# robjermy/CMVS-PMVS

Hardware: AMD Instinct MI355X
Metric: refined patches/sec + NCC evals/sec, 50-view 4K synthetic, 1/2/4/8 GPU (higher is better)
Workload: dtype f32 (f64 optimizer)

## Files before the change

cmvs-pmvs_amd/csrc/bobyqa_dev.h:

```cpp
#pragma once

#if defined(__HIPCC__)
#define BQ_HD __host__ __device__ inline __attribute__((always_inline))
#else
#define BQ_HD inline
#endif
#if defined(__HIP_DEVICE_COMPILE__) && defined(BQ_PRIVATE)
#define BQ_AS __attribute__((address_space(5)))
#elif defined(__HIP_DEVICE_COMPILE__)
#define BQ_AS __attribute__((address_space(3)))
#else
#define BQ_AS
#endif
#if defined(__HIPCC__) && !defined(BQ_INLINE)
#define BQ_NI __host__ __device__ inline __attribute__((noinline))
#else
#define BQ_NI BQ_HD
#endif

#include <math.h>

#if defined(BQ_NO_RESTRICT)
#define BQ_RS
#else
// ... 37 lines not shown
BQ_HD double bq_min(double a, double b) { return (a <= b) ? a : b; }
BQ_HD double bq_max(double a, double b) { return (a >= b) ? a : b; }
template <int N>
BQ_HD double bq_get(const double (&a)[N], int i) {
  double r = a[0];
#pragma unroll
  for (int k = 1; k < N; ++k) r = (i == k) ? a[k] : r;
  return r;
}
template <int N>
BQ_HD void bq_set(double (&a)[N], int i, double v) {
#pragma unroll
  for (int k = 0; k < N; ++k) a[k] = (i == k) ? v : a[k];
}

struct BqState {
  double x_[BQN], xl_[BQN], xu_[BQN], s[BQN];
  double rhobeg, rhoend;
  int maxeval, nevals;
  double xbase_[BQN], xpt_[BQNPT][BQN], fval_[BQNPT], xopt_[BQN], gopt_[BQN], hq_[BQNH], pq_[BQNPT],
      bmat_[BQNDIM][BQN], zmat_[BQNPT][BQNPTM], sl_[BQN], su_[BQN], xnew_[BQN], xalt_[BQN], d_[BQN],
      vlag_[BQNDIM], w_[BQNDIM + BQNPT];
  double gnew_[BQN];
  double ptsaux_[2][BQN], ptsid_[BQNPT];
  double f, fbeg, fsave, xoptsq, rho, delta, diffa, diffb, diffc, dnorm, distsq, dsq, crvmin,
      adelt, alpha, cauchy, beta, denom, fopt, vquad, diff, ratio, stepa, stepb;
  int nf, kopt, kbase, nresc, ntrits, itest, nfsav, knew;
  int nfm, nfx, kpt, rs_ip, rs_iq;
  double rs_xp, rs_xq, rs_vq, rs_fbase;
  int rc;
  int resume;
  double xeval[BQN];
  double xout[BQN];
  double minf;
};

#define BQ_A1(name) BQ_AS double* const name = (st).name##_ - 1
#define BQ_A2(name, C) BQ_AS double(*const name)[C] = (BQ_AS double(*)[C])(&(st).name##_[0][0] - (C) - 1)
#define BQ_ALIASES(st)                                                                                         \
  BQ_A1(x); BQ_A1(xl); BQ_A1(xu); BQ_A1(xbase); BQ_A1(fval); BQ_A1(xopt); BQ_A1(gopt); BQ_A1(hq); BQ_A1(pq); \
  BQ_A1(sl); BQ_A1(su); BQ_A1(xnew); BQ_A1(xalt); BQ_A1(d); BQ_A1(vlag); BQ_A1(w); BQ_A1(gnew); BQ_A1(ptsid); \
  BQ_A2(xpt, BQN); BQ_A2(bmat, BQN); BQ_A2(zmat, BQNPTM); BQ_A2(ptsaux, BQN)

BQ_NI void bq_trsbox(const BQ_AS double (*BQ_RST xpt)[BQN], const BQ_AS double* BQ_RST xopt_m, const BQ_AS double* BQ_RST gopt,
                     const BQ_AS double* BQ_RST hq_m, const BQ_AS double* BQ_RST pq_m, const BQ_AS double* BQ_RST sl_m,
                     const BQ_AS double* BQ_RST su_m, double delta, BQ_AS double* BQ_RST xnew, BQ_AS double* BQ_RST d_m,
                     BQ_AS double* BQ_RST gnew_m, BQ_AS double* BQ_RST dsq_out, BQ_AS double* BQ_RST crvmin_out) {
  const double half = 0.5, one = 1.0, onemin = -1.0, zero = 0.0;
#if !defined(BQ_TRSBOX_LDS)
  double xopt[BQN + 1], hq[BQNH + 1], pq[BQNPT + 1], sl[BQN + 1], su[BQN + 1], d[BQN + 1], gnew[BQN + 1];
  for (int k = 1; k <= BQNPT; ++k) pq[k] = pq_m[k];
  for (int i = 1; i <= BQNH; ++i) hq[i] = hq_m[i];
  for (int i = 1; i <= BQN; ++i) {
    xopt[i] = xopt_m[i];
    sl[i] = sl_m[i];
    su[i] = su_m[i];
  }
// ... 550 lines not shown

BQ_HD double bq_default_step(double x, double lb, double ub) {
  double step = HUGE_VAL;
  if (!isinf(ub) && !isinf(lb) && (ub - lb) * 0.25 < step && ub > lb) step = (ub - lb) * 0.25;
  if (!isinf(ub) && ub - x < step && ub > x) step = (ub - x) * 0.75;
  if (!isinf(lb) && x - lb < step && x > lb) step = (x - lb) * 0.75;
  if (isinf(step)) {
    if (!isinf(ub) && fabs(ub - x) < fabs(step)) step = (ub - x) * 1.1;
    if (!isinf(lb) && fabs(x - lb) < fabs(step)) step = (x - lb) * 1.1;
  }
  if (isinf(step) || step == 0.0 || fabs(step) < 2.2250738585072014e-308) step = x;
  if (isinf(step) || step == 0.0) step = 1;
  return step;
}

BQ_HD int bq_begin(BQ_AS BqState& st, const double* x0, const double* lb, const double* ub,
                   double xtol_rel, int maxeval) {
  BQ_ALIASES(st);
  double dxs[BQN];
  for (int i = 0; i < BQN; ++i) dxs[i] = bq_default_step(x0[i], lb[i], ub[i]);
  for (int i = 0; i < BQN; ++i) st.s[i] = 1.0;
  {
    int i = 1;
    for (; i < BQN && dxs[i] == dxs[i - 1]; ++i) {
    }
    if (i < BQN)
      for (i = 1; i < BQN; ++i) st.s[i] = dxs[i] / dxs[0];
  }
  for (int i = 0; i < BQN; ++i) {
    x[i + 1] = x0[i] / st.s[i];
    xl[i + 1] = lb[i] / st.s[i];
    xu[i + 1] = ub[i] / st.s[i];
  }
  st.rhobeg = fabs(dxs[0] / st.s[0]);
  st.rhoend = xtol_rel * st.rhobeg;
  st.maxeval = maxeval;
  st.nevals = 0;
  st.rc = BQR_SUCCESS;
  st.resume = 0;
  st.minf = 0;
  for (int j = 1; j <= BQN; ++j) {
    const double temp = xu[j] - xl[j];
    if (temp < st.rhobeg + st.rhobeg) {
      st.rc = BQR_INVALID_ARGS;
      for (int i = 0; i < BQN; ++i) st.xout[i] = x0[i];
      st.resume = -1;
      return BQR_INVALID_ARGS;
    }
    sl[j] = xl[j] - x[j];
    su[j] = xu[j] - x[j];
    if (sl[j] >= -st.rhobeg) {
      if (sl[j] >= 0.0) {
        x[j] = xl[j];
        sl[j] = 0.0;
        su[j] = temp;
      } else {
        x[j] = xl[j] + st.rhobeg;
        sl[j] = -st.rhobeg;
        su[j] = bq_max(xu[j] - x[j], st.rhobeg);
      }
    } else if (su[j] <= st.rhobeg) {
      if (su[j] <= 0.0) {
        x[j] = xu[j];
        sl[j] = -temp;
        su[j] = 0.0;
      } else {
        x[j] = xu[j] - st.rhobeg;
        sl[j] = bq_min(xl[j] - x[j], -st.rhobeg);
        su[j] = st.rhobeg;
      }
    }
  }
  return 0;
}

#define BQ_CALFUN(P, LABEL_ID)                                             \
  do {                                                                     \
    for (int i_ = 0; i_ < BQN; ++i_) st.xeval[i_] = (P)[i_ + 1] * st.s[i_]; \
    st.nevals++;                                                           \
    st.resume = LABEL_ID;                                                  \
    return BQ_NEED_F;                                                      \
  } while (0)

BQ_NI int bq_step_impl(BQ_AS BqState& st, double fin);
BQ_HD int bq_step(BQ_AS BqState& st, double fin) {
  BQ_PT(t_all);
  const int r = bq_step_impl(st, fin);
  BQ_PA(3, t_all);
  return r;
}
BQ_NI int bq_step_impl(BQ_AS BqState& st, double fin) {
  BQ_ALIASES(st);
  const double half = 0.5, one = 1.0, ten = 10.0, tenth = 0.1, two = 2.0, zero = 0.0;
  double temp, sum, suma, sumb, bsum, dx, delsq, scaden, biglsq, hdiag, den, errbig, frhosq,
      bdtol, bdtest, curv, fracsq, sumpq, sumz, sumw, densav, pqold, gqsq, gisq, dist;
  int ih, ksav;
  switch (st.resume) {
    case 0: goto PSTART;
    case 1: goto PRESUME;
    case 2: goto L360R;
    case 3: goto R260R;
    default: return BQ_DONE;
  }
PSTART: {
    for (int j = 1; j <= BQN; ++j) {
      xbase[j] = x[j];
      for (int k = 1; k <= BQNPT; ++k) xpt[k][j] = zero;
      for (int i = 1; i <= BQNDIM; ++i) bmat[i][j] = zero;
    }
    for (int i = 1; i <= BQNH; ++i) hq[i] = zero;
    for (int k = 1; k <= BQNPT; ++k) {
      pq[k] = zero;
      for (int j = 1; j <= BQNPTM; ++j) zmat[k][j] = zero;
    }
    st.nf = 0;
    st.kopt = 1;
  PLOOP:
    st.nfm = st.nf;
    st.nfx = st.nf - BQN;
    ++st.nf;
    if (st.nfm <= 2 * BQN) {
      if (st.nfm >= 1 && st.nfm <= BQN) {
        st.stepa = st.rhobeg;
        if (su[st.nfm] == zero) st.stepa = -st.stepa;
        xpt[st.nf][st.nfm] = st.stepa;
      } else if (st.nfm > BQN) {
        st.stepa = xpt[st.nf - BQN][st.nfx];
        st.stepb = -st.rhobeg;
        if (sl[st.nfx] == zero) st.stepb = bq_min(two * st.rhobeg, su[st.nfx]);
        if (su[st.nfx] == zero) st.stepb = bq_max(-two * st.rhobeg, sl[st.nfx]);
        xpt[st.nf][st.nfx] = st.stepb;
      }
    }
    for (int j = 1; j <= BQN; ++j) {
      x[j] = bq_min(bq_max(xl[j], xbase[j] + xpt[st.nf][j]), xu[j]);
      if (xpt[st.nf][j] == sl[j]) x[j] = xl[j];
      if (xpt[st.nf][j] == su[j]) x[j] = xu[j];
    }
    BQ_CALFUN(x, 1);
  }
PRESUME: {
    const double rhosq = st.rhobeg * st.rhobeg;
    const int nf = st.nf, nfm = st.nfm, nfx = st.nfx;
    st.f = fin;
    fval[nf] = st.f;
    if (nf == 1) {
      st.fbeg = st.f;
      st.kopt = 1;
    } else if (st.f < fval[st.kopt]) {
      st.kopt = nf;
    }
    if (nf <= 2 * BQN + 1) {
      if (nf >= 2 && nf <= BQN + 1) {
        gopt[nfm] = (st.f - st.fbeg) / st.stepa;
        if (BQNPT < nf + BQN) {
          bmat[1][nfm] = -one / st.stepa;
          bmat[nf][nfm] = one / st.stepa;
          bmat[BQNPT + nfm][nfm] = -half * rhosq;
        }
      } else if (nf >= BQN + 2) {
        ih = nfx * (nfx + 1) / 2;
        temp = (st.f - st.fbeg) / st.stepb;
        st.diff = st.stepb - st.stepa;
        hq[ih] = two * (temp - gopt[nfx]) / st.diff;
        gopt[nfx] = (gopt[nfx] * st.stepb - temp * st.stepa) / st.diff;
        if (st.stepa * st.stepb < zero) {
          if (st.f < fval[nf - BQN]) {
            fval[nf] = fval[nf - BQN];
            fval[nf - BQN] = st.f;
            if (st.kopt == nf) st.kopt = nf - BQN;
            xpt[nf - BQN][nfx] = st.stepb;
            xpt[nf][nfx] = st.stepa;
          }
        }
        bmat[1][nfx] = -(st.stepa + st.stepb) / (st.stepa * st.stepb);
        bmat[nf][nfx] = -half / xpt[nf - BQN][nfx];
        bmat[nf - BQN][nfx] = -bmat[1][nfx] - bmat[nf][nfx];
        zmat[1][nfx] = sqrt(two) / (st.stepa * st.stepb);
        zmat[nf][nfx] = sqrt(half) / rhosq;
        zmat[nf - BQN][nfx] = -zmat[1][nfx] - zmat[nf][nfx];
      }
    }
    if (st.maxeval > 0 && st.nevals >= st.maxeval) {
      st.rc = BQR_MAXEVAL;
    } else if (st.nf < BQNPT) {
      goto PLOOP;
    }
  }
  st.xoptsq = zero;
  for (int i = 1; i <= BQN; ++i) {
    xopt[i] = xpt[st.kopt][i];
    st.xoptsq += xopt[i] * xopt[i];
  }
  st.fsave = fval[1];
  if (st.rc != BQR_SUCCESS) goto L720;
  st.kbase = 1;
  st.rho = st.rhobeg;
  st.delta = st.rho;
  st.nresc = st.nf;
  st.ntrits = 0;
  st.diffa = zero;
  st.diffb = zero;
  st.diffc = zero;
  st.ratio = zero;
  st.itest = 0;
  st.nfsav = st.nf;
  st.knew = 0;
L20:
  if (st.kopt != st.kbase) {
    ih = 0;
    for (int j = 1; j <= BQN; ++j) {
      for (int i = 1; i <= j; ++i) {
// ... 139 lines not shown
    for (int j = 1; j <= BQN; ++j) {
      xbase[j] += xopt[j];
      sl[j] -= xopt[j];
      su[j] -= xopt[j];
      xopt[j] = zero;
      ptsaux[1][j] = bq_min(st.delta, su[j]);
      ptsaux[2][j] = bq_max(-st.delta, sl[j]);
      if (ptsaux[1][j] + ptsaux[2][j] < zero) {
        temp = ptsaux[1][j];
        ptsaux[1][j] = ptsaux[2][j];
        ptsaux[2][j] = temp;
      }
      if (fabs(ptsaux[2][j]) < half * fabs(ptsaux[1][j])) ptsaux[2][j] = half * ptsaux[1][j];
      for (int i = 1; i <= BQNDIM; ++i) bmat[i][j] = zero;
    }
    st.rs_fbase = fval[st.kopt];
    ptsid[1] = sfrac;
    for (int j = 1; j <= BQN; ++j) {
      const int jp = j + 1, jpn = jp + BQN;
      ptsid[jp] = (double)j + sfrac;
      if (jpn <= BQNPT) {
        ptsid[jpn] = (double)j / (double)BQNP + sfrac;
        temp = one / (ptsaux[1][j] - ptsaux[2][j]);
        bmat[jp][j] = -temp + one / ptsaux[1][j];
        bmat[jpn][j] = temp + one / ptsaux[2][j];
        bmat[1][j] = -bmat[jp][j] - bmat[jpn][j];
        zmat[1][j] = sqrt(2.) / fabs(ptsaux[1][j] * ptsaux[2][j]);
        zmat[jp][j] = zmat[1][j] * ptsaux[2][j] * temp;
        zmat[jpn][j] = -zmat[1][j] * ptsaux[1][j] * temp;
      } else {
        bmat[1][j] = -one / ptsaux[1][j];
// ... 91 lines not shown
        den = bet2 * hdiag + vlag[k] * vlag[k];
        if (den > den2) {
          kold = k;
          den2 = den;
        }
      }
      vlmxsq = bq_max(vlmxsq, vlag[k] * vlag[k]);
    }
    if (den2 <= vlmxsq * .01) {
      w[BQNDIM + kn] = -w[BQNDIM + kn] - winc;
      goto R120;
    }
    goto R80;
  }
R260:
  st.kpt = 1;
R260LOOP:
  if (st.kpt > BQNPT) goto R350;
  if (ptsid[st.kpt] == zero) {
    ++st.kpt;
    goto R260LOOP;
  }
  if (st.maxeval > 0 && st.nevals >= st.maxeval) {
    st.nf = -1;
    goto R350;
  }
  {
    const int kpt = st.kpt;
    ih = 0;
    for (int j = 1; j <= BQN; ++j) {
      w[j] = xpt[kpt][j];
      xpt[kpt][j] = zero;
      temp = pq[kpt] * w[j];
      for (int i = 1; i <= j; ++i) {
        ++ih;
        hq[ih] += temp * w[i];
      }
    }
    pq[kpt] = zero;
    st.rs_ip = (int)ptsid[kpt];
    st.rs_iq = (int)((double)BQNP * ptsid[kpt] - (double)(st.rs_ip * BQNP));
    const int ip = st.rs_ip, iq = st.rs_iq;
    int ihp = 0, ihq;
    if (ip > 0) {
      st.rs_xp = ptsaux[1][ip];
      xpt[kpt][ip] = st.rs_xp;
    }
    if (iq > 0) {
      st.rs_xq = ptsaux[1][iq];
      if (ip == 0) st.rs_xq = ptsaux[2][iq];
      xpt[kpt][iq] = st.rs_xq;
    }
    st.rs_vq = st.rs_fbase;
    if (ip > 0) {
      ihp = (ip + ip * ip) / 2;
      st.rs_vq += st.rs_xp * (gopt[ip] + half * st.rs_xp * hq[ihp]);
    }
    if (iq > 0) {
      ihq = (iq + iq * iq) / 2;
      st.rs_vq += st.rs_xq * (gopt[iq] + half * st.rs_xq * hq[ihq]);
      if (ip > 0) {
        const int iw = (ihp > ihq ? ihp : ihq) - (ip > iq ? ip - iq : iq - ip);
        st.rs_vq += st.rs_xp * st.rs_xq * hq[iw];
      }
    }
    for (int k = 1; k <= BQNPT; ++k) {
      temp = zero;
      if (ip > 0) temp += st.rs_xp * xpt[k][ip];
      if (iq > 0) temp += st.rs_xq * xpt[k][iq];
      st.rs_vq += half * pq[k] * temp * temp;
    }
    for (int i = 1; i <= BQN; ++i) {
      w[i] = bq_min(bq_max(xl[i], xbase[i] + xpt[kpt][i]), xu[i]);
      if (xpt[kpt][i] == sl[i]) w[i] = xl[i];
      if (xpt[kpt][i] == su[i]) w[i] = xu[i];
    }
    ++st.nf;
    BQ_CALFUN(w, 3);
  }
R260R: {
    const int kpt = st.kpt, ip0 = st.rs_ip, iq0 = st.rs_iq;
    (void)ip0; (void)iq0;
    st.f = fin;
    fval[kpt] = st.f;
    if (st.f < fval[st.kopt]) st.kopt = kpt;
    st.diff = st.f - st.rs_vq;
    for (int i = 1; i <= BQN; ++i) gopt[i] += st.diff * bmat[kpt][i];
    for (int k = 1; k <= BQNPT; ++k) {
      sum = zero;
      for (int j = 1; j <= BQNPTM; ++j) sum += zmat[k][j] * zmat[kpt][j];
      temp = st.diff * sum;
      if (ptsid[k] == zero) {
        pq[k] += temp;
      } else {
        const int ip = (int)ptsid[k];
        const int iq = (int)((double)BQNP * ptsid[k] - (double)(ip * BQNP));
        const int ihq = (iq * iq + iq) / 2;
        if (ip == 0) {
          hq[ihq] += temp * (ptsaux[2][iq] * ptsaux[2][iq]);
        } else {
          const int ihp = (ip * ip + ip) / 2;
          hq[ihp] += temp * (ptsaux[1][ip] * ptsaux[1][ip]);
          if (iq > 0) {
            hq[ihq] += temp * (ptsaux[1][iq] * ptsaux[1][iq]);
            const int iw = (ihp > ihq ? ihp : ihq) - (iq > ip ? iq - ip : ip - iq);
            hq[iw] += temp * ptsaux[1][ip] * ptsaux[1][iq];
          }
        }
      }
    }
    ptsid[kpt] = zero;
    ++st.kpt;
    goto R260LOOP;
  }
R350:
  st.xoptsq = zero;
  if (st.kopt != st.kbase) {
    for (int i = 1; i <= BQN; ++i) {
      xopt[i] = xpt[st.kopt][i];
      st.xoptsq += xopt[i] * xopt[i];
    }
  }
  if (st.nf < 0) {
    st.nf = st.maxeval;
    st.rc = BQR_MAXEVAL;
    goto L720;
  }
// ... 99 lines not shown
    if (xnew[i] == sl[i]) x[i] = xl[i];
    if (xnew[i] == su[i]) x[i] = xu[i];
  }
  if (st.maxeval > 0 && st.nevals >= st.maxeval) {
    st.rc = BQR_MAXEVAL;
    goto L720;
  }
  ++st.nf;
  BQ_CALFUN(x, 2);
L360R:
  st.f = fin;
  if (st.ntrits == -1) {
    st.fsave = st.f;
    st.rc = BQR_XTOL;
    if (st.fsave < fval[st.kopt]) {
      st.minf = st.f;
      for (int i = 0; i < BQN; ++i) st.xout[i] = x[i + 1] * st.s[i];
      st.resume = -1;
      return BQ_DONE;
    }
    goto L720;
  }
  st.fopt = fval[st.kopt];
  st.vquad = zero;
  ih = 0;
  for (int j = 1; j <= BQN; ++j) {
    st.vquad += d[j] * gopt[j];
    for (int i = 1; i <= j; ++i) {
      ++ih;
      temp = d[i] * d[j];
      if (i == j) temp = half * temp;
      st.vquad += hq[ih] * temp;
// ... 195 lines not shown
    st.ntrits = 0;
    st.nfsav = st.nf;
    goto L60;
  }
  if (st.ntrits == -1) goto L360;
  st.rc = BQR_XTOL;
L720:
  if (fval[st.kopt] <= st.fsave) {
    for (int i = 1; i <= BQN; ++i) {
      x[i] = bq_min(bq_max(xl[i], xbase[i] + xopt[i]), xu[i]);
      if (xopt[i] == sl[i]) x[i] = xl[i];
      if (xopt[i] == su[i]) x[i] = xu[i];
    }
    st.f = fval[st.kopt];
  }
  st.minf = st.f;
  for (int i = 0; i < BQN; ++i) st.xout[i] = x[i + 1] * st.s[i];
  st.resume = -1;
  return BQ_DONE;
}

#undef BQ_CALFUN

}
```

cmvs-pmvs_amd/csrc/pmvs_api.cpp:

```cpp
#include <hip/hip_runtime.h>

#include <algorithm>
#include <climits>
#include <cmath>
#include <cstdarg>
#include <cstdio>
#include <cstdlib>
#include <cstring>
#include <chrono>
#include <condition_variable>
#include <mutex>
#include <string>
#include <vector>

#include "../../include/pmvs_amd.h"
#include "pmvs_features.h"
#include "pmvs_fmt.h"
#include "pmvs_launch.h"

using namespace pmvsdev;

namespace {

thread_local std::string g_err = "";
// ... 125 lines not shown
  DScene ds{};
  int maxLevel = 0;
  std::vector<DView> hviews;
  DevBuf<DView> views;
  DevBuf<uint32_t> pyr;
  DevBuf<uint8_t> masks, edges;
  DevBuf<int> vis_off, vis, bindexes;
  DevBuf<float> scratch;
  DevBuf<DevStats> stats;
  DevBuf<RefineJob> jobs;
  FilterBuffers fbuf;
  ExpandBuffers xbuf;
  DevBuf<pmvs_patch> fpatches;
  DevBuf<int> fkeep;
  DevBuf<unsigned long long> digest;
  int grid = 0, refine_grid = 0, tslots = 226014;
  int tslots_small = 300000, small_n = 7000;
  int refine_cfg(int n) const { return n < small_n ? tslots_small : tslots; }
  int shard_rank = 0, shard_world = 1;
  pmvs_allgather_fn shard_fn = nullptr;
  void* shard_ctx = nullptr;
  pmvs_rccl* shard_rccl = nullptr;
  int cl_rank = 0, cl_world = 1;
  pmvs_allgather_fn cl_fn = nullptr;
  void* cl_ctx = nullptr;
  pmvs_rccl* cl_rccl = nullptr;
  DevBuf<unsigned char> cl_shared;
  DevBuf<int> cl_ids, cl_id2idx;
  int cl_maxid = -1;
  ClusterBuffers cbuf;
  RefineHost rhost;
// ... 1631 lines not shown
```

cmvs-pmvs_amd/csrc/pmvs_kernels.hip:

```cpp
#include <hip/hip_runtime.h>

#include <algorithm>
#include <cmath>
#include <condition_variable>
#include <functional>
#include <mutex>
#include <thread>
#include <unistd.h>
#include <vector>

#include "bobyqa_dev.h"
#include "pmvs_device.h"
#include "pmvs_refine.h"

namespace pmvsdev {

#ifndef REFINE_TSLOTS
#define REFINE_TSLOTS 48
#endif

typedef uint16_t img_t;

template <int WS>
struct WaveLds {
// ... 1664 lines not shown
    if ((e = launch_refine_lane(tslots, s, d_jobs, n, d_st, stream)) != hipSuccess) return e;
    if (refine_tail_on()) hipLaunchKernelGGL(refine_tail_kernel, dim3(1), dim3(64), 0, stream, d_st, 1);
    (void)hipEventRecord(ev[2], stream);
    hipLaunchKernelGGL((post_kernel<WS>), dim3(g), dim3(64), 0, stream, s, d_jobs, d_out, n, d_st);
    (void)hipEventRecord(ev[3], stream);
    return hipGetLastError();
  }
  if (tslots >= 200000 && tslots < 300000 && WS > 7) tslots = 1206;
  if (tslots / 100 < s.tau) {
    tslots = 2408;
    refine_grid = refine_grid / 2 > 0 ? refine_grid / 2 : 1;
  }
  const int nc = tslots % 100;
  const int rg = refine_grid < (n + nc - 1) / nc ? refine_grid : (n + nc - 1) / nc;
  if (tslots >= 200000) {
    if ((e = launch_refine_split(tslots, s, d_jobs, n, d_st, stream)) != hipSuccess) return e;
    if (refine_tail_on()) hipLaunchKernelGGL(refine_tail_kernel, dim3(1), dim3(64), 0, stream, d_st, 0);
    (void)hipEventRecord(ev[2], stream);
    hipLaunchKernelGGL((post_kernel<WS>), dim3(g), dim3(64), 0, stream, s, d_jobs, d_out, n, d_st);
    (void)hipEventRecord(ev[3], stream);
    dump_jobs(d_jobs, n, stream);
    return hipGetLastError();
  }
  if (tslots >= 100000) {
    const int ncw = (tslots / 1000) % 100, wgpc = tslots % 10;
    int dev = 0, cus = 0;
    if ((e = hipGetDevice(&dev)) != hipSuccess ||
        (e = hipDeviceGetAttribute(&cus, hipDeviceAttributeMultiprocessorCount, dev)) != hipSuccess)
      return e;
    cus = cus > 0 ? cus : 1;
    const int wgrid = cus * wgpc < n ? cus * wgpc : n;
// ... 408 lines not shown
```

cmvs-pmvs_amd/csrc/pmvs_launch.h:

```cpp
#pragma once
#include <hip/hip_runtime.h>
#include "pmvs_device.h"
#include "pmvs_devbuf.h"
#include <functional>
#include <memory>
#include <utility>
#include <vector>

namespace pmvsdev {

inline hipError_t memset_big(void* p, int value, size_t bytes, hipStream_t st) {
  constexpr size_t kPiece = size_t(1) << 30;
  char* c = static_cast<char*>(p);
  for (size_t off = 0; off < bytes; off += kPiece) {
    const hipError_t e = hipMemsetAsync(c + off, value, bytes - off < kPiece ? bytes - off : kPiece, st);
    if (e != hipSuccess) return e;
  }
  return hipSuccess;
}
bool refine_config_supported(int tslots);
struct RefineHost {
  float4* d_enc = nullptr;
  double2* d_ang = nullptr;
  float4* h_enc = nullptr;
  double2* h_ang = nullptr;
  size_t cap = 0;
  bool prof = false;
  hipEvent_t ev_pre = nullptr;
  double trip_ms = 0.0;
  long long trips = 0;
  hipError_t ensure(size_t n);
  void release();
  ~RefineHost() { release(); }
};
int prepost_waves();
hipError_t launch_refine(const DScene& s, const pmvs_candidate* d_in, RefineJob* d_jobs, pmvs_refined* d_out, int n,
                         DevStats* d_st, int grid, int refine_grid, int tslots, hipStream_t stream, hipEvent_t* ev,
                         RefineHost& rh);
bool refine_split_supported(int config);
hipError_t launch_refine_split(int config, const DScene& s, RefineJob* d_jobs, int n, DevStats* d_st, hipStream_t stream);
bool refine_lane_supported(int config);
hipError_t launch_refine_lane(int config, const DScene& s, RefineJob* d_jobs, int n, DevStats* d_st, hipStream_t stream);
hipError_t launch_incc_eval(const DScene& s, const pmvs_eval_query* d_q, int n, double* d_out, DevStats* d_st,
                            hipStream_t stream);
hipError_t launch_grab_tex(const DScene& s, const pmvs_tex_query* d_q, int n, float* d_out, int* d_valid,
                           hipStream_t stream);
hipError_t launch_build_level(const uint8_t* d_src, int Wp, int Hp, uint8_t* d_dst, int W, int H, hipStream_t stream);
hipError_t launch_pack_rgba(const uint8_t* d_rgb, uint32_t* d_out, long long npix, hipStream_t stream);
hipError_t launch_unpack_rgba(const uint32_t* d_in, uint8_t* d_rgb, long long npix, hipStream_t stream);
hipError_t launch_math_selftest(int op, const double* d_in, double* d_out, int n, hipStream_t stream);
hipError_t launch_bobyqa_selftest(int mode, int kind, const double* d_x0, int n, int maxeval, double* d_out,
                                  hipStream_t stream);
hipError_t launch_model_digest(const void* recs, int n, int record_bytes, unsigned long long* d_out, hipStream_t stream);
hipError_t launch_patch_colors(const DScene& s, int n, const float* coords, const int* off, const int* images, int* out,
                               hipStream_t stream);
// ... 216 lines not shown
```

cmvs-pmvs_amd/csrc/pmvs_refine_split.hip:

```cpp
#include <hip/hip_runtime.h>

#include "bobyqa_dev.h"
#include "pmvs_device.h"
#include "pmvs_launch.h"
#include "pmvs_refine.h"

namespace pmvsdev {

#if defined(BQ_PROFILE)
#define SP_NOW() __builtin_amdgcn_s_memtime()
#define SP_MARK(slot)                                      \
  do {                                                     \
    const unsigned long long _t = __builtin_amdgcn_s_memtime(); \
    prof[slot] += _t - tprev;                              \
    tprev = _t;                                            \
  } while (0)
#else
#define SP_NOW() 0ull
#define SP_MARK(slot) \
  do {                \
  } while (0)
#endif

#ifndef SPLIT_WPE
#define SPLIT_WPE 2
#endif
#ifndef SPLIT_THREADS_
#define SPLIT_THREADS_ 512
#endif
constexpr int SPLIT_THREADS = SPLIT_THREADS_;
constexpr int SPLIT_TS = 64;

template <int WS, int G, int CG>
struct RefSplitLds {
  static constexpr int NCH = G * CG;
  static constexpr int SLOTS = CG * PMVS_MAX_TAU;
  BqState bq[NCH];
  float geo[NCH][16];
  double fv[NCH];
  int cand[NCH];
  unsigned short views[NCH][PMVS_MAX_TAU];
  unsigned char need[NCH], size[NCH];
  unsigned char sreq[G][SLOTS], sidx[G][SLOTS];
  short choff[G][CG + 1];
  int nchunk[G];
  int avail[G], done[G];
  int live;
  int ejvalid[8][SPLIT_TS];
  float ejres[8][SPLIT_TS];
};

#define SPLIT_AS __attribute__((address_space(3)))
// ... 186 lines not shown
    C.fv[cc] = request_value(s, V, t, C.size[cc], need, jobs[C.cand[cc]], tex_valid);
  }
  SP_MARK(6);
  __builtin_amdgcn_fence(__ATOMIC_RELEASE, "workgroup");
  if (lane == 0) __hip_atomic_fetch_add(&C.done[g], 1, __ATOMIC_RELEASE, __HIP_MEMORY_SCOPE_WORKGROUP);
  return tex_valid;
}
template <int WS, int G, int CG, int LP>
__device__ __noinline__ unsigned long long split_chunk(const DScene& s, SPLIT_AS RefSplitLds<WS, G, CG>& C,
                                                       RefineJob* __restrict__ jobs, int g, int k, unsigned long long* prof) {
  return split_chunk_body<WS, G, CG, LP>(s, C, jobs, g, k, prof);
}

template <int WS, int G, int CG, int LP>
__device__ __noinline__ void split_optimizer(const DScene& s, SPLIT_AS RefSplitLds<WS, G, CG>& C, RefineJob* __restrict__ jobs,
                                             int n, int nc_active, DevStats* st) {
  constexpr int TS = WAVE / LP;
  const int wave = threadIdx.x >> 6, lane = threadIdx.x & (WAVE - 1);
  const int g = wave;
  const bool owner = lane < CG && lane < nc_active;
  const int c = g * CG + (lane < CG ? lane : 0);
  BQ_AS BqState& bq = *(BQ_AS BqState*)&C.bq[c];
  RefineSetup R;
  int cand = -1, need = 0, evals = 0, size = 0, nimg = 0, rc = 0;
  bool exhausted = !owner;
  double fv = 0.0;
  float fcoord[4], fnormal[4];
  unsigned long long nevals = 0, rounds = 0, tex_valid = 0, grabs = 0, chunks = 0;
  const double lb[3] = {-HUGE_VAL, -23.99999, -23.99999};
  const double ub[3] = {HUGE_VAL, 23.99999, 23.99999};
  unsigned long long prof[8] = {0, 0, 0, 0, 0, 0, 0, 0};
  unsigned long long tprev = SP_NOW();
  for (;;) {
    while (cand < 0 && !exhausted) {
      const unsigned long long q = atomicAdd(&st->queue2, 1ull);
      if (q >= (unsigned long long)n) {
        exhausted = true;
// ... 1 lines not shown
        break;
      }
      const RefineJob& J = jobs[q];
      if (J.status != PMVS_ACCEPTED) continue;
      cand = (int)q;
      for (int i = 0; i < 4; ++i) { R.center[i] = J.center[i]; R.ray[i] = J.ray[i]; }
      R.dscale = J.dscale;
      R.ascale = s.ascale;
      R.ref = J.images[0];
      nimg = J.nimg;
      size = imin(s.tau, nimg);
      for (int i = 0; i < size; ++i) C.views[c][i] = (unsigned short)J.images[i];
      C.cand[c] = cand;
      evals = 0;
      const double x0[3] = {J.x0[0], J.x0[1], J.x0[2]};
      bq_begin(bq, x0, lb, ub, 1.e-7, 1000);
      fv = 0.0;
      need = 0;
    }
    SP_MARK(0);
    if (cand >= 0 && need == 0) {
      const int r = (bq.resume < 0) ? BQ_DONE : bq_step(bq, fv);
      if (r == BQ_NEED_F) {
        need = 1;
        const double xe[3] = {bq.xeval[0], bq.xeval[1], bq.xeval[2]};
        decode(s, R, xe, fcoord, fnormal);
      } else {
        rc = bq.rc;
        const bool success = (rc == BQR_SUCCESS || rc == 2 || rc == 3 || rc == BQR_XTOL);
        RefineJob& J = jobs[cand];
        J.refine_code = rc;
        J.evals = evals;
        if (success) {
          const double xo[3] = {bq.xout[0], bq.xout[1], bq.xout[2]};
          decode(s, R, xo, fcoord, fnormal);
          if (nimg < 2) {
            J.ncc = (float)(1.0 - (double)unrobustincc(2.0f));
            for (int i = 0; i < 4; ++i) { J.rcoord[i] = fcoord[i]; J.rnormal[i] = fnormal[i]; }
            cand = -1;
          } else {
            need = 2;
          }
        } else {
          cand = -1;
        }
      }
    }
    SP_MARK(1);
    const bool req = (cand >= 0 && need != 0);
// ... 129 lines not shown
  }
  SP_MARK(7);
  for (int d = 32; d >= 1; d >>= 1) tex_valid += __shfl_xor(tex_valid, d);
  if (lane == 0) {
#if defined(BQ_PROFILE)
    for (int i = 4; i < 8; ++i) atomicAdd(&st->prof[i], prof[i]);
#endif
    atomicAdd(&st->tex_valid, tex_valid);
    atomicAdd(&st->tex_grabs, grabs);
    atomicAdd(&st->chunks, chunks);
  }
}

template <int WS, int G, int CG, int LP>
__global__ __launch_bounds__(SPLIT_THREADS) __attribute__((amdgpu_waves_per_eu(SPLIT_WPE))) void refine_split_kernel(
    DScene s, RefineJob* __restrict__ jobs, int n, int nc_active, DevStats* st) {
  using L = RefSplitLds<WS, G, CG>;
  static_assert(G >= 1 && G <= SPLIT_THREADS / WAVE && CG <= WAVE && CG <= 255, "roles");
  static_assert(sizeof(L) <= 160 * 1024, "LDS");
  __shared__ L C;
  const int tid = threadIdx.x, wave = tid >> 6;
  if (tid < G) {
    C.avail[tid] = 0;
    C.done[tid] = 0;
    C.nchunk[tid] = 0;
  }
  if (tid == 0) {
    C.live = G;
    atomicMax(&st->t_first_inv, ~__builtin_amdgcn_s_memrealtime());
  }
  __syncthreads();
  if (wave < G)
    split_optimizer<WS, G, CG, LP>(s, *(SPLIT_AS RefSplitLds<WS, G, CG>*)&C, jobs, n, nc_active, st);
  else
    split_evaluator<WS, G, CG, LP>(s, *(SPLIT_AS RefSplitLds<WS, G, CG>*)&C, jobs, st);
}


#if SPLIT_THREADS_ == 512
#define PMVS_SPLIT_CONFIGS(X) X(0, 2, 32) X(0, 4, 16) X(2, 4, 16) X(2, 5, 16) X(2, 6, 12) X(2, 6, 14) X(2, 7, 12) \
  X(2, 8, 10) X(3, 6, 14) X(4, 5, 16) X(4, 6, 14) X(4, 7, 12) X(4, 8, 10) X(8, 8, 10)
#else
#define PMVS_SPLIT_CONFIGS(X) X(2, 4, 20) X(4, 4, 20) X(8, 4, 20) X(2, 2, 40) X(4, 3, 24)
#endif
bool refine_split_supported(int config) {
#define PMVS_SPLIT_CASE(LPc, Gc, CGc) case 200000 + LPc * 10000 + Gc * 1000 + CGc:
  switch (config) {
    PMVS_SPLIT_CONFIGS(PMVS_SPLIT_CASE)
    return true;
    default: return false;
  }
#undef PMVS_SPLIT_CASE
}

template <int WS>
static hipError_t launch_split_ws(int config, const DScene& s, RefineJob* d_jobs, int n, DevStats* d_st, hipStream_t stream) {
  const int gw = (config / 1000) % 10, cg = config % 1000;
  int dev = 0, cus = 0;
  hipError_t e;
  if ((e = hipGetDevice(&dev)) != hipSuccess ||
      (e = hipDeviceGetAttribute(&cus, hipDeviceAttributeMultiprocessorCount, dev)) != hipSuccess)
    return e;
  cus = cus > 0 ? cus : 1;
  const int sgrid = cus < (n + gw - 1) / gw ? cus : (n + gw - 1) / gw;
  const int per = (n + sgrid * gw - 1) / (sgrid * gw);
  const int nca = per < cg ? per : cg;
#define PMVS_SPLIT_LAUNCH(LPc, Gc, CGc)                                                                                   \
  case 200000 + LPc * 10000 + Gc * 1000 + CGc:                                                                             \
    hipLaunchKernelGGL((refine_split_kernel<WS, Gc, CGc, (LPc > 0 ? LPc : 1)>), dim3(sgrid), dim3(SPLIT_THREADS), 0, stream, \
                       s, d_jobs, n, nca, d_st);                                                                           \
    break;
  switch (config) {
    PMVS_SPLIT_CONFIGS(PMVS_SPLIT_LAUNCH)
    default: return hipErrorInvalidValue;
  }
#undef PMVS_SPLIT_LAUNCH
  return hipGetLastError();
}

hipError_t launch_refine_split(int config, const DScene& s, RefineJob* d_jobs, int n, DevStats* d_st, hipStream_t stream) {
  if (n <= 0) return hipSuccess;
  switch (s.wsize) {
    case 5: return launch_split_ws<5>(config, s, d_jobs, n, d_st, stream);
    case 7: return launch_split_ws<7>(config, s, d_jobs, n, d_st, stream);
    default: return hipErrorInvalidValue;
  }
}

}
```

Measured before the change: 949,000.

## Split BOBYQA state into LDS-resident hot part and global cold part

Splits the per-chain optimizer state into a hot struct kept in LDS and a cold struct (rhobeg, rescue scratch, output) moved to a global buffer sized per CU. Shrinking per-chain LDS lets more chains fit per block, and the default split config changes from 2-6-14 to 2-5-19, one of several newly added configs. Rarely used fields now incur global memory traffic, and the host grows a device buffer before each launch.

```diff
diff --git a/cmvs-pmvs_amd/csrc/bobyqa_dev.h b/cmvs-pmvs_amd/csrc/bobyqa_dev.h
--- a/cmvs-pmvs_amd/csrc/bobyqa_dev.h
+++ b/cmvs-pmvs_amd/csrc/bobyqa_dev.h
@@ -75,33 +75,43 @@
   for (int k = 0; k < N; ++k) a[k] = (i == k) ? v : a[k];
 }
 
-struct BqState {
+struct BqHot {
   double x_[BQN], xl_[BQN], xu_[BQN], s[BQN];
-  double rhobeg, rhoend;
+  double rhoend;
   int maxeval, nevals;
   double xbase_[BQN], xpt_[BQNPT][BQN], fval_[BQNPT], xopt_[BQN], gopt_[BQN], hq_[BQNH], pq_[BQNPT],
       bmat_[BQNDIM][BQN], zmat_[BQNPT][BQNPTM], sl_[BQN], su_[BQN], xnew_[BQN], xalt_[BQN], d_[BQN],
       vlag_[BQNDIM], w_[BQNDIM + BQNPT];
   double gnew_[BQN];
-  double ptsaux_[2][BQN], ptsid_[BQNPT];
-  double f, fbeg, fsave, xoptsq, rho, delta, diffa, diffb, diffc, dnorm, distsq, dsq, crvmin,
-      adelt, alpha, cauchy, beta, denom, fopt, vquad, diff, ratio, stepa, stepb;
+  double f, fsave, xoptsq, rho, delta, diffa, diffb, diffc, dnorm, distsq, dsq, crvmin,
+      adelt, alpha, cauchy, beta, denom, fopt, vquad, diff, ratio;
   int nf, kopt, kbase, nresc, ntrits, itest, nfsav, knew;
-  int nfm, nfx, kpt, rs_ip, rs_iq;
-  double rs_xp, rs_xq, rs_vq, rs_fbase;
   int rc;
   int resume;
   double xeval[BQN];
+};
+struct BqCold {
+  double rhobeg;
+  double fbeg, stepa, stepb;
+  double ptsaux_[2][BQN], ptsid_[BQNPT];
+  int nfm, nfx, kpt, rs_ip, rs_iq;
+  double rs_xp, rs_xq, rs_vq, rs_fbase;
   double xout[BQN];
   double minf;
 };
+struct BqState : BqHot, BqCold {};
+static_assert(sizeof(BqHot) <= 1512, "BqHot: the hot optimizer state of a chain");
+static_assert(sizeof(BqState) == sizeof(BqHot) + sizeof(BqCold), "BqState is BqHot and BqCold, nothing else");
 
 #define BQ_A1(name) BQ_AS double* const name = (st).name##_ - 1
 #define BQ_A2(name, C) BQ_AS double(*const name)[C] = (BQ_AS double(*)[C])(&(st).name##_[0][0] - (C) - 1)
 #define BQ_ALIASES(st)                                                                                         \
   BQ_A1(x); BQ_A1(xl); BQ_A1(xu); BQ_A1(xbase); BQ_A1(fval); BQ_A1(xopt); BQ_A1(gopt); BQ_A1(hq); BQ_A1(pq); \
-  BQ_A1(sl); BQ_A1(su); BQ_A1(xnew); BQ_A1(xalt); BQ_A1(d); BQ_A1(vlag); BQ_A1(w); BQ_A1(gnew); BQ_A1(ptsid); \
-  BQ_A2(xpt, BQN); BQ_A2(bmat, BQN); BQ_A2(zmat, BQNPTM); BQ_A2(ptsaux, BQN)
+  BQ_A1(sl); BQ_A1(su); BQ_A1(xnew); BQ_A1(xalt); BQ_A1(d); BQ_A1(vlag); BQ_A1(w); BQ_A1(gnew);               \
+  BQ_A2(xpt, BQN); BQ_A2(bmat, BQN); BQ_A2(zmat, BQNPTM)
+#define BQ_COLD_ALIASES(cs)                        \
+  auto* const ptsid = &(cs).ptsid_[0] - 1;         \
+  auto* const ptsaux = (decltype(&(cs).ptsaux_[0]))(&(cs).ptsaux_[0][0] - BQN - 1)
 
 BQ_NI void bq_trsbox(const BQ_AS double (*BQ_RST xpt)[BQN], const BQ_AS double* BQ_RST xopt_m, const BQ_AS double* BQ_RST gopt,
                      const BQ_AS double* BQ_RST hq_m, const BQ_AS double* BQ_RST pq_m, const BQ_AS double* BQ_RST sl_m,
@@ -682,7 +692,8 @@
   return step;
 }
 
-BQ_HD int bq_begin(BQ_AS BqState& st, const double* x0, const double* lb, const double* ub,
+template <class CT>
+BQ_HD int bq_begin(BQ_AS BqHot& st, CT& cs, const double* x0, const double* lb, const double* ub,
                    double xtol_rel, int maxeval) {
   BQ_ALIASES(st);
   double dxs[BQN];
@@ -700,42 +711,42 @@
     xl[i + 1] = lb[i] / st.s[i];
     xu[i + 1] = ub[i] / st.s[i];
   }
-  st.rhobeg = fabs(dxs[0] / st.s[0]);
-  st.rhoend = xtol_rel * st.rhobeg;
+  cs.rhobeg = fabs(dxs[0] / st.s[0]);
+  st.rhoend = xtol_rel * cs.rhobeg;
   st.maxeval = maxeval;
   st.nevals = 0;
   st.rc = BQR_SUCCESS;
   st.resume = 0;
-  st.minf = 0;
+  cs.minf = 0;
   for (int j = 1; j <= BQN; ++j) {
     const double temp = xu[j] - xl[j];
-    if (temp < st.rhobeg + st.rhobeg) {
+    if (temp < cs.rhobeg + cs.rhobeg) {
       st.rc = BQR_INVALID_ARGS;
-      for (int i = 0; i < BQN; ++i) st.xout[i] = x0[i];
+      for (int i = 0; i < BQN; ++i) cs.xout[i] = x0[i];
       st.resume = -1;
       return BQR_INVALID_ARGS;
     }
     sl[j] = xl[j] - x[j];
     su[j] = xu[j] - x[j];
-    if (sl[j] >= -st.rhobeg) {
+    if (sl[j] >= -cs.rhobeg) {
       if (sl[j] >= 0.0) {
         x[j] = xl[j];
         sl[j] = 0.0;
         su[j] = temp;
       } else {
-        x[j] = xl[j] + st.rhobeg;
-        sl[j] = -st.rhobeg;
-        su[j] = bq_max(xu[j] - x[j], st.rhobeg);
-      }
-    } else if (su[j] <= st.rhobeg) {
+        x[j] = xl[j] + cs.rhobeg;
+        sl[j] = -cs.rhobeg;
+        su[j] = bq_max(xu[j] - x[j], cs.rhobeg);
+      }
+    } else if (su[j] <= cs.rhobeg) {
       if (su[j] <= 0.0) {
         x[j] = xu[j];
         sl[j] = -temp;
         su[j] = 0.0;
       } else {
-        x[j] = xu[j] - st.rhobeg;
-        sl[j] = bq_min(xl[j] - x[j], -st.rhobeg);
-        su[j] = st.rhobeg;
+        x[j] = xu[j] - cs.rhobeg;
+        sl[j] = bq_min(xl[j] - x[j], -cs.rhobeg);
+        su[j] = cs.rhobeg;
       }
     }
   }
@@ -750,15 +761,29 @@
     return BQ_NEED_F;                                                      \
   } while (0)
 
-BQ_NI int bq_step_impl(BQ_AS BqState& st, double fin);
-BQ_HD int bq_step(BQ_AS BqState& st, double fin) {
+struct BqColdInState {};
+BQ_HD BQ_AS BqCold& bq_cold(BQ_AS BqHot& st, BqColdInState) { return static_cast<BQ_AS BqState&>(st); }
+template <class CT>
+BQ_HD CT& bq_cold(BQ_AS BqHot&, CT* cp) { return *cp; }
+
+template <class CP>
+BQ_NI int bq_step_impl(BQ_AS BqHot& st, CP cp, double fin);
+template <class CP>
+BQ_HD int bq_step(BQ_AS BqHot& st, CP cp, double fin) {
   BQ_PT(t_all);
-  const int r = bq_step_impl(st, fin);
+  const int r = bq_step_impl(st, cp, fin);
   BQ_PA(3, t_all);
   return r;
 }
-BQ_NI int bq_step_impl(BQ_AS BqState& st, double fin) {
+BQ_HD int bq_begin(BQ_AS BqState& st, const double* x0, const double* lb, const double* ub, double xtol_rel, int maxeval) {
+  return bq_begin(static_cast<BQ_AS BqHot&>(st), static_cast<BQ_AS BqCold&>(st), x0, lb, ub, xtol_rel, maxeval);
+}
+BQ_HD int bq_step(BQ_AS BqState& st, double fin) { return bq_step(static_cast<BQ_AS BqHot&>(st), BqColdInState{}, fin); }
+template <class CP>
+BQ_NI int bq_step_impl(BQ_AS BqHot& st, CP cp, double fin) {
+  auto& cs = bq_cold(st, cp);
   BQ_ALIASES(st);
+  BQ_COLD_ALIASES(cs);
   const double half = 0.5, one = 1.0, ten = 10.0, tenth = 0.1, two = 2.0, zero = 0.0;
   double temp, sum, suma, sumb, bsum, dx, delsq, scaden, biglsq, hdiag, den, errbig, frhosq,
       bdtol, bdtest, curv, fracsq, sumpq, sumz, sumw, densav, pqold, gqsq, gisq, dist;
@@ -784,20 +809,20 @@
     st.nf = 0;
     st.kopt = 1;
   PLOOP:
-    st.nfm = st.nf;
-    st.nfx = st.nf - BQN;
+    cs.nfm = st.nf;
+    cs.nfx = st.nf - BQN;
     ++st.nf;
-    if (st.nfm <= 2 * BQN) {
-      if (st.nfm >= 1 && st.nfm <= BQN) {
-        st.stepa = st.rhobeg;
-        if (su[st.nfm] == zero) st.stepa = -st.stepa;
-        xpt[st.nf][st.nfm] = st.stepa;
-      } else if (st.nfm > BQN) {
-        st.stepa = xpt[st.nf - BQN][st.nfx];
-        st.stepb = -st.rhobeg;
-        if (sl[st.nfx] == zero) st.stepb = bq_min(two * st.rhobeg, su[st.nfx]);
-        if (su[st.nfx] == zero) st.stepb = bq_max(-two * st.rhobeg, sl[st.nfx]);
-        xpt[st.nf][st.nfx] = st.stepb;
+    if (cs.nfm <= 2 * BQN) {
+      if (cs.nfm >= 1 && cs.nfm <= BQN) {
+        cs.stepa = cs.rhobeg;
+        if (su[cs.nfm] == zero) cs.stepa = -cs.stepa;
+        xpt[st.nf][cs.nfm] = cs.stepa;
+      } else if (cs.nfm > BQN) {
+        cs.stepa = xpt[st.nf - BQN][cs.nfx];
+        cs.stepb = -cs.rhobeg;
+        if (sl[cs.nfx] == zero) cs.stepb = bq_min(two * cs.rhobeg, su[cs.nfx]);
+        if (su[cs.nfx] == zero) cs.stepb = bq_max(-two * cs.rhobeg, sl[cs.nfx]);
+        xpt[st.nf][cs.nfx] = cs.stepb;
       }
     }
     for (int j = 1; j <= BQN; ++j) {
@@ -808,43 +833,43 @@
     BQ_CALFUN(x, 1);
   }
 PRESUME: {
-    const double rhosq = st.rhobeg * st.rhobeg;
-    const int nf = st.nf, nfm = st.nfm, nfx = st.nfx;
+    const double rhosq = cs.rhobeg * cs.rhobeg;
+    const int nf = st.nf, nfm = cs.nfm, nfx = cs.nfx;
     st.f = fin;
     fval[nf] = st.f;
     if (nf == 1) {
-      st.fbeg = st.f;
+      cs.fbeg = st.f;
       st.kopt = 1;
     } else if (st.f < fval[st.kopt]) {
       st.kopt = nf;
     }
     if (nf <= 2 * BQN + 1) {
       if (nf >= 2 && nf <= BQN + 1) {
-        gopt[nfm] = (st.f - st.fbeg) / st.stepa;
+        gopt[nfm] = (st.f - cs.fbeg) / cs.stepa;
         if (BQNPT < nf + BQN) {
-          bmat[1][nfm] = -one / st.stepa;
-          bmat[nf][nfm] = one / st.stepa;
+          bmat[1][nfm] = -one / cs.stepa;
+          bmat[nf][nfm] = one / cs.stepa;
           bmat[BQNPT + nfm][nfm] = -half * rhosq;
         }
       } else if (nf >= BQN + 2) {
         ih = nfx * (nfx + 1) / 2;
-        temp = (st.f - st.fbeg) / st.stepb;
-        st.diff = st.stepb - st.stepa;
+        temp = (st.f - cs.fbeg) / cs.stepb;
+        st.diff = cs.stepb - cs.stepa;
         hq[ih] = two * (temp - gopt[nfx]) / st.diff;
-        gopt[nfx] = (gopt[nfx] * st.stepb - temp * st.stepa) / st.diff;
-        if (st.stepa * st.stepb < zero) {
+        gopt[nfx] = (gopt[nfx] * cs.stepb - temp * cs.stepa) / st.diff;
+        if (cs.stepa * cs.stepb < zero) {
           if (st.f < fval[nf - BQN]) {
             fval[nf] = fval[nf - BQN];
             fval[nf - BQN] = st.f;
             if (st.kopt == nf) st.kopt = nf - BQN;
-            xpt[nf - BQN][nfx] = st.stepb;
-            xpt[nf][nfx] = st.stepa;
+            xpt[nf - BQN][nfx] = cs.stepb;
+            xpt[nf][nfx] = cs.stepa;
           }
         }
-        bmat[1][nfx] = -(st.stepa + st.stepb) / (st.stepa * st.stepb);
+        bmat[1][nfx] = -(cs.stepa + cs.stepb) / (cs.stepa * cs.stepb);
         bmat[nf][nfx] = -half / xpt[nf - BQN][nfx];
         bmat[nf - BQN][nfx] = -bmat[1][nfx] - bmat[nf][nfx];
-        zmat[1][nfx] = sqrt(two) / (st.stepa * st.stepb);
+        zmat[1][nfx] = sqrt(two) / (cs.stepa * cs.stepb);
         zmat[nf][nfx] = sqrt(half) / rhosq;
         zmat[nf - BQN][nfx] = -zmat[1][nfx] - zmat[nf][nfx];
       }
@@ -863,7 +888,7 @@
   st.fsave = fval[1];
   if (st.rc != BQR_SUCCESS) goto L720;
   st.kbase = 1;
-  st.rho = st.rhobeg;
+  st.rho = cs.rhobeg;
   st.delta = st.rho;
   st.nresc = st.nf;
   st.ntrits = 0;
@@ -1033,7 +1058,7 @@
       if (fabs(ptsaux[2][j]) < half * fabs(ptsaux[1][j])) ptsaux[2][j] = half * ptsaux[1][j];
       for (int i = 1; i <= BQNDIM; ++i) bmat[i][j] = zero;
     }
-    st.rs_fbase = fval[st.kopt];
+    cs.rs_fbase = fval[st.kopt];
     ptsid[1] = sfrac;
     for (int j = 1; j <= BQN; ++j) {
       const int jp = j + 1, jpn = jp + BQN;
@@ -1155,11 +1180,11 @@
     goto R80;
   }
 R260:
-  st.kpt = 1;
+  cs.kpt = 1;
 R260LOOP:
-  if (st.kpt > BQNPT) goto R350;
-  if (ptsid[st.kpt] == zero) {
-    ++st.kpt;
+  if (cs.kpt > BQNPT) goto R350;
+  if (ptsid[cs.kpt] == zero) {
+    ++cs.kpt;
     goto R260LOOP;
   }
   if (st.maxeval > 0 && st.nevals >= st.maxeval) {
@@ -1167,7 +1192,7 @@
     goto R350;
   }
   {
-    const int kpt = st.kpt;
+    const int kpt = cs.kpt;
     ih = 0;
     for (int j = 1; j <= BQN; ++j) {
       w[j] = xpt[kpt][j];
@@ -1179,37 +1204,37 @@
       }
     }
     pq[kpt] = zero;
-    st.rs_ip = (int)ptsid[kpt];
-    st.rs_iq = (int)((double)BQNP * ptsid[kpt] - (double)(st.rs_ip * BQNP));
-    const int ip = st.rs_ip, iq = st.rs_iq;
+    cs.rs_ip = (int)ptsid[kpt];
+    cs.rs_iq = (int)((double)BQNP * ptsid[kpt] - (double)(cs.rs_ip * BQNP));
+    const int ip = cs.rs_ip, iq = cs.rs_iq;
     int ihp = 0, ihq;
     if (ip > 0) {
-      st.rs_xp = ptsaux[1][ip];
-      xpt[kpt][ip] = st.rs_xp;
+      cs.rs_xp = ptsaux[1][ip];
+      xpt[kpt][ip] = cs.rs_xp;
     }
     if (iq > 0) {
-      st.rs_xq = ptsaux[1][iq];
-      if (ip == 0) st.rs_xq = ptsaux[2][iq];
-      xpt[kpt][iq] = st.rs_xq;
-    }
-    st.rs_vq = st.rs_fbase;
+      cs.rs_xq = ptsaux[1][iq];
+      if (ip == 0) cs.rs_xq = ptsaux[2][iq];
+      xpt[kpt][iq] = cs.rs_xq;
+    }
+    cs.rs_vq = cs.rs_fbase;
     if (ip > 0) {
       ihp = (ip + ip * ip) / 2;
-      st.rs_vq += st.rs_xp * (gopt[ip] + half * st.rs_xp * hq[ihp]);
+      cs.rs_vq += cs.rs_xp * (gopt[ip] + half * cs.rs_xp * hq[ihp]);
     }
     if (iq > 0) {
       ihq = (iq + iq * iq) / 2;
-      st.rs_vq += st.rs_xq * (gopt[iq] + half * st.rs_xq * hq[ihq]);
+      cs.rs_vq += cs.rs_xq * (gopt[iq] + half * cs.rs_xq * hq[ihq]);
       if (ip > 0) {
         const int iw = (ihp > ihq ? ihp : ihq) - (ip > iq ? ip - iq : iq - ip);
-        st.rs_vq += st.rs_xp * st.rs_xq * hq[iw];
+        cs.rs_vq += cs.rs_xp * cs.rs_xq * hq[iw];
       }
     }
     for (int k = 1; k <= BQNPT; ++k) {
       temp = zero;
-      if (ip > 0) temp += st.rs_xp * xpt[k][ip];
-      if (iq > 0) temp += st.rs_xq * xpt[k][iq];
-      st.rs_vq += half * pq[k] * temp * temp;
+      if (ip > 0) temp += cs.rs_xp * xpt[k][ip];
+      if (iq > 0) temp += cs.rs_xq * xpt[k][iq];
+      cs.rs_vq += half * pq[k] * temp * temp;
     }
     for (int i = 1; i <= BQN; ++i) {
       w[i] = bq_min(bq_max(xl[i], xbase[i] + xpt[kpt][i]), xu[i]);
@@ -1220,12 +1245,12 @@
     BQ_CALFUN(w, 3);
   }
 R260R: {
-    const int kpt = st.kpt, ip0 = st.rs_ip, iq0 = st.rs_iq;
+    const int kpt = cs.kpt, ip0 = cs.rs_ip, iq0 = cs.rs_iq;
     (void)ip0; (void)iq0;
     st.f = fin;
     fval[kpt] = st.f;
     if (st.f < fval[st.kopt]) st.kopt = kpt;
-    st.diff = st.f - st.rs_vq;
+    st.diff = st.f - cs.rs_vq;
     for (int i = 1; i <= BQN; ++i) gopt[i] += st.diff * bmat[kpt][i];
     for (int k = 1; k <= BQNPT; ++k) {
       sum = zero;
@@ -1251,7 +1276,7 @@
       }
     }
     ptsid[kpt] = zero;
-    ++st.kpt;
+    ++cs.kpt;
     goto R260LOOP;
   }
 R350:
@@ -1381,8 +1406,8 @@
     st.fsave = st.f;
     st.rc = BQR_XTOL;
     if (st.fsave < fval[st.kopt]) {
-      st.minf = st.f;
-      for (int i = 0; i < BQN; ++i) st.xout[i] = x[i + 1] * st.s[i];
+      cs.minf = st.f;
+      for (int i = 0; i < BQN; ++i) cs.xout[i] = x[i + 1] * st.s[i];
       st.resume = -1;
       return BQ_DONE;
     }
@@ -1608,8 +1633,8 @@
     }
     st.f = fval[st.kopt];
   }
-  st.minf = st.f;
-  for (int i = 0; i < BQN; ++i) st.xout[i] = x[i + 1] * st.s[i];
+  cs.minf = st.f;
+  for (int i = 0; i < BQN; ++i) cs.xout[i] = x[i + 1] * st.s[i];
   st.resume = -1;
   return BQ_DONE;
 }
diff --git a/cmvs-pmvs_amd/csrc/pmvs_api.cpp b/cmvs-pmvs_amd/csrc/pmvs_api.cpp
--- a/cmvs-pmvs_amd/csrc/pmvs_api.cpp
+++ b/cmvs-pmvs_amd/csrc/pmvs_api.cpp
@@ -163,7 +163,7 @@
   DevBuf<pmvs_patch> fpatches;
   DevBuf<int> fkeep;
   DevBuf<unsigned long long> digest;
-  int grid = 0, refine_grid = 0, tslots = 226014;
+  int grid = 0, refine_grid = 0, tslots = 225019;
   int tslots_small = 300000, small_n = 7000;
   int refine_cfg(int n) const { return n < small_n ? tslots_small : tslots; }
   int shard_rank = 0, shard_world = 1;
diff --git a/cmvs-pmvs_amd/csrc/pmvs_kernels.hip b/cmvs-pmvs_amd/csrc/pmvs_kernels.hip
--- a/cmvs-pmvs_amd/csrc/pmvs_kernels.hip
+++ b/cmvs-pmvs_amd/csrc/pmvs_kernels.hip
@@ -1702,7 +1702,7 @@
   const int nc = tslots % 100;
   const int rg = refine_grid < (n + nc - 1) / nc ? refine_grid : (n + nc - 1) / nc;
   if (tslots >= 200000) {
-    if ((e = launch_refine_split(tslots, s, d_jobs, n, d_st, stream)) != hipSuccess) return e;
+    if ((e = launch_refine_split(tslots, s, d_jobs, n, d_st, stream, rh.bq_cold)) != hipSuccess) return e;
     if (refine_tail_on()) hipLaunchKernelGGL(refine_tail_kernel, dim3(1), dim3(64), 0, stream, d_st, 0);
     (void)hipEventRecord(ev[2], stream);
     hipLaunchKernelGGL((post_kernel<WS>), dim3(g), dim3(64), 0, stream, s, d_jobs, d_out, n, d_st);
diff --git a/cmvs-pmvs_amd/csrc/pmvs_launch.h b/cmvs-pmvs_amd/csrc/pmvs_launch.h
--- a/cmvs-pmvs_amd/csrc/pmvs_launch.h
+++ b/cmvs-pmvs_amd/csrc/pmvs_launch.h
@@ -25,6 +25,7 @@
   float4* h_enc = nullptr;
   double2* h_ang = nullptr;
   size_t cap = 0;
+  DevBuf<unsigned char> bq_cold;
   bool prof = false;
   hipEvent_t ev_pre = nullptr;
   double trip_ms = 0.0;
@@ -38,7 +39,8 @@
                          DevStats* d_st, int grid, int refine_grid, int tslots, hipStream_t stream, hipEvent_t* ev,
                          RefineHost& rh);
 bool refine_split_supported(int config);
-hipError_t launch_refine_split(int config, const DScene& s, RefineJob* d_jobs, int n, DevStats* d_st, hipStream_t stream);
+hipError_t launch_refine_split(int config, const DScene& s, RefineJob* d_jobs, int n, DevStats* d_st, hipStream_t stream,
+                               DevBuf<unsigned char>& cold);
 bool refine_lane_supported(int config);
 hipError_t launch_refine_lane(int config, const DScene& s, RefineJob* d_jobs, int n, DevStats* d_st, hipStream_t stream);
 hipError_t launch_incc_eval(const DScene& s, const pmvs_eval_query* d_q, int n, double* d_out, DevStats* d_st,
diff --git a/cmvs-pmvs_amd/csrc/pmvs_refine_split.hip b/cmvs-pmvs_amd/csrc/pmvs_refine_split.hip
--- a/cmvs-pmvs_amd/csrc/pmvs_refine_split.hip
+++ b/cmvs-pmvs_amd/csrc/pmvs_refine_split.hip
@@ -35,7 +35,7 @@
 struct RefSplitLds {
   static constexpr int NCH = G * CG;
   static constexpr int SLOTS = CG * PMVS_MAX_TAU;
-  BqState bq[NCH];
+  BqHot bq[NCH];
   float geo[NCH][16];
   double fv[NCH];
   int cand[NCH];
@@ -252,13 +252,14 @@
 
 template <int WS, int G, int CG, int LP>
 __device__ __noinline__ void split_optimizer(const DScene& s, SPLIT_AS RefSplitLds<WS, G, CG>& C, RefineJob* __restrict__ jobs,
-                                             int n, int nc_active, DevStats* st) {
+                                             BqCold* __restrict__ cold, int n, int nc_active, DevStats* st) {
   constexpr int TS = WAVE / LP;
   const int wave = threadIdx.x >> 6, lane = threadIdx.x & (WAVE - 1);
   const int g = wave;
   const bool owner = lane < CG && lane < nc_active;
   const int c = g * CG + (lane < CG ? lane : 0);
-  BQ_AS BqState& bq = *(BQ_AS BqState*)&C.bq[c];
+  BQ_AS BqHot& bq = *(BQ_AS BqHot*)&C.bq[c];
+  BqCold& bc = cold[(size_t)blockIdx.x * (G * CG) + c];
   RefineSetup R;
   int cand = -1, need = 0, evals = 0, size = 0, nimg = 0, rc = 0;
   bool exhausted = !owner;
@@ -290,13 +291,13 @@
       C.cand[c] = cand;
       evals = 0;
       const double x0[3] = {J.x0[0], J.x0[1], J.x0[2]};
-      bq_begin(bq, x0, lb, ub, 1.e-7, 1000);
+      bq_begin(bq, bc, x0, lb, ub, 1.e-7, 1000);
       fv = 0.0;
       need = 0;
     }
     SP_MARK(0);
     if (cand >= 0 && need == 0) {
-      const int r = (bq.resume < 0) ? BQ_DONE : bq_step(bq, fv);
+      const int r = (bq.resume < 0) ? BQ_DONE : bq_step(bq, &bc, fv);
       if (r == BQ_NEED_F) {
         need = 1;
         const double xe[3] = {bq.xeval[0], bq.xeval[1], bq.xeval[2]};
@@ -308,7 +309,7 @@
         J.refine_code = rc;
         J.evals = evals;
         if (success) {
-          const double xo[3] = {bq.xout[0], bq.xout[1], bq.xout[2]};
+          const double xo[3] = {bc.xout[0], bc.xout[1], bc.xout[2]};
           decode(s, R, xo, fcoord, fnormal);
           if (nimg < 2) {
             J.ncc = (float)(1.0 - (double)unrobustincc(2.0f));
@@ -468,7 +469,7 @@
 
 template <int WS, int G, int CG, int LP>
 __global__ __launch_bounds__(SPLIT_THREADS) __attribute__((amdgpu_waves_per_eu(SPLIT_WPE))) void refine_split_kernel(
-    DScene s, RefineJob* __restrict__ jobs, int n, int nc_active, DevStats* st) {
+    DScene s, RefineJob* __restrict__ jobs, BqCold* __restrict__ cold, int n, int nc_active, DevStats* st) {
   using L = RefSplitLds<WS, G, CG>;
   static_assert(G >= 1 && G <= SPLIT_THREADS / WAVE && CG <= WAVE && CG <= 255, "roles");
   static_assert(sizeof(L) <= 160 * 1024, "LDS");
@@ -485,15 +486,15 @@
   }
   __syncthreads();
   if (wave < G)
-    split_optimizer<WS, G, CG, LP>(s, *(SPLIT_AS RefSplitLds<WS, G, CG>*)&C, jobs, n, nc_active, st);
+    split_optimizer<WS, G, CG, LP>(s, *(SPLIT_AS RefSplitLds<WS, G, CG>*)&C, jobs, cold, n, nc_active, st);
   else
     split_evaluator<WS, G, CG, LP>(s, *(SPLIT_AS RefSplitLds<WS, G, CG>*)&C, jobs, st);
 }
 
 
 #if SPLIT_THREADS_ == 512
-#define PMVS_SPLIT_CONFIGS(X) X(0, 2, 32) X(0, 4, 16) X(2, 4, 16) X(2, 5, 16) X(2, 6, 12) X(2, 6, 14) X(2, 7, 12) \
-  X(2, 8, 10) X(3, 6, 14) X(4, 5, 16) X(4, 6, 14) X(4, 7, 12) X(4, 8, 10) X(8, 8, 10)
+#define PMVS_SPLIT_CONFIGS(X) X(0, 2, 32) X(0, 4, 16) X(2, 4, 16) X(2, 5, 16) X(2, 5, 19) X(2, 6, 12) X(2, 6, 14) X(2, 6, 15) \
+  X(2, 6, 16) X(2, 7, 12) X(2, 7, 13) X(2, 8, 10) X(3, 6, 14) X(4, 5, 16) X(4, 6, 14) X(4, 7, 12) X(4, 8, 10) X(8, 8, 10)
 #else
 #define PMVS_SPLIT_CONFIGS(X) X(2, 4, 20) X(4, 4, 20) X(8, 4, 20) X(2, 2, 40) X(4, 3, 24)
 #endif
@@ -508,7 +509,8 @@
 }
 
 template <int WS>
-static hipError_t launch_split_ws(int config, const DScene& s, RefineJob* d_jobs, int n, DevStats* d_st, hipStream_t stream) {
+static hipError_t launch_split_ws(int config, const DScene& s, RefineJob* d_jobs, int n, DevStats* d_st, hipStream_t stream,
+                                  DevBuf<unsigned char>& cold) {
   const int gw = (config / 1000) % 10, cg = config % 1000;
   int dev = 0, cus = 0;
   hipError_t e;
@@ -519,10 +521,11 @@
   const int sgrid = cus < (n + gw - 1) / gw ? cus : (n + gw - 1) / gw;
   const int per = (n + sgrid * gw - 1) / (sgrid * gw);
   const int nca = per < cg ? per : cg;
+  if ((e = cold.grow((size_t)cus * gw * cg * sizeof(BqCold))) != hipSuccess) return e;
 #define PMVS_SPLIT_LAUNCH(LPc, Gc, CGc)                                                                                   \
   case 200000 + LPc * 10000 + Gc * 1000 + CGc:                                                                             \
     hipLaunchKernelGGL((refine_split_kernel<WS, Gc, CGc, (LPc > 0 ? LPc : 1)>), dim3(sgrid), dim3(SPLIT_THREADS), 0, stream, \
-                       s, d_jobs, n, nca, d_st);                                                                           \
+                       s, d_jobs, (BqCold*)cold.p, n, nca, d_st);                                                          \
     break;
   switch (config) {
     PMVS_SPLIT_CONFIGS(PMVS_SPLIT_LAUNCH)
@@ -532,11 +535,12 @@
   return hipGetLastError();
 }
 
-hipError_t launch_refine_split(int config, const DScene& s, RefineJob* d_jobs, int n, DevStats* d_st, hipStream_t stream) {
+hipError_t launch_refine_split(int config, const DScene& s, RefineJob* d_jobs, int n, DevStats* d_st, hipStream_t stream,
+                               DevBuf<unsigned char>& cold) {
   if (n <= 0) return hipSuccess;
   switch (s.wsize) {
-    case 5: return launch_split_ws<5>(config, s, d_jobs, n, d_st, stream);
-    case 7: return launch_split_ws<7>(config, s, d_jobs, n, d_st, stream);
+    case 5: return launch_split_ws<5>(config, s, d_jobs, n, d_st, stream, cold);
+    case 7: return launch_split_ws<7>(config, s, d_jobs, n, d_st, stream, cold);
     default: return hipErrorInvalidValue;
   }
 }
```

After: 961,100 (median of 6 runs). 1.3% higher.
